# bcsefercik/markerless-robot-camera-calibration

Measured on AMD Instinct MI355X. Metric: point-cloud frames/sec at 200k pts/frame, higher is better.
Workload: dtype f32

## Files before the change

### include/sv_hip.h

```cpp
#ifndef SV_HIP_H
#define SV_HIP_H

#include <stddef.h>
#include <stdint.h>

#ifdef __cplusplus
extern "C" {
#endif

#define SV_OK 0
#define SV_ERR_INVALID (-1)
#define SV_ERR_WORKSPACE (-2)
#define SV_ERR_HIP (-3)
#define SV_ERR_RANGE (-4)
#define SV_ERR_UNSUPPORTED (-5)

#define SV_ACT_NONE 0
#define SV_ACT_RELU 1
#define SV_ACT_LEAKY_RELU 2

#define SV_POOL_MAX 0
#define SV_POOL_AVG 1

#define SV_REDUCE_MEAN 0
#define SV_REDUCE_FIRST 1

#define SV_TILE_ROWS 128
#define SV_COORD_BIAS 131072
#define SV_COORD_BITS 18
#define SV_MAX_BATCH 1024

typedef void* sv_stream_t;

const char* sv_last_error(void);
#define SV_ABI_VERSION 4
int sv_abi_version(void);

size_t sv_voxelize_workspace_bytes(int64_t N);
int sv_voxelize(const void* coords4, int coords_are_int, int64_t N, void* workspace, size_t workspace_bytes,
                uint64_t* keys, int32_t* vcoords, int64_t* inverse, int32_t* order, int32_t* seg_start,
                int32_t* counters, sv_stream_t stream);

int sv_voxel_reduce(const float* feats, int C, const int32_t* order, const int32_t* seg_start, int64_t V, int mode,
                    float* out, sv_stream_t stream);

int sv_hash_build(const uint64_t* keys, int64_t V, uint64_t* table_keys, int32_t* table_vals, int64_t capacity,
                  sv_stream_t stream);

size_t sv_stride_map_workspace_bytes(int64_t V_in);
int sv_stride_map(const uint64_t* keys_in, int64_t V_in, int level, void* workspace, size_t workspace_bytes,
                  uint64_t* keys_out, int32_t* vcoords_out, int32_t* parent, int32_t* child_start, int32_t* counters,
                  sv_stream_t stream);

int sv_kernel_map_k3(const int32_t* vcoords, int64_t V, int tensor_stride, int dilation, const uint64_t* table_keys,
                     const int32_t* table_vals, int64_t capacity, int32_t* nbr, int64_t ld, uint32_t* mask,
                     sv_stream_t stream);
int sv_kernel_map_down(const uint64_t* keys_fine, const int32_t* parent, int64_t V_fine, int level, int64_t V_coarse,
                       int32_t* nbr, int64_t ld, uint32_t* mask, sv_stream_t stream);
int sv_kernel_map_up(const uint64_t* keys_fine, const int32_t* parent, int64_t V_fine, int level, int32_t* nbr,
                     int64_t ld, uint32_t* mask, sv_stream_t stream);

size_t sv_plan_workspace_bytes(int64_t V);
int sv_plan_build(const int32_t* nbr, int64_t ld, const uint32_t* mask, int K, int64_t V, int64_t nbr_base, void* workspace,
                  size_t workspace_bytes, int32_t* perm, int32_t* nbr_s, uint32_t* submask, int32_t* tile_order,
                  int64_t Vpad, sv_stream_t stream);

#define SV_FRAME_MAX_LEVELS 8
#define SV_FRAME_MAX_CUTS 4
#define SV_FRAME_K3 1
#define SV_FRAME_DOWN 2
#define SV_FRAME_UP 4
#define SV_FRAME_SPLIT 8
#define SV_FRAME_RECORD 16
#define SV_FRAME_REC_HASH 1
#define SV_FRAME_REC_K3 2
#define SV_FRAME_REC_DOWN 3
#define SV_FRAME_REC_UP 4
#define SV_FRAME_REC_SPLIT 5
size_t sv_frame_maps_arena_bytes(int64_t N, int levels);
size_t sv_frame_maps_scratch_bytes(int64_t N);
int sv_frame_maps(const void* coords4, int coords_are_int, int64_t N, int levels, void* arena, size_t arena_bytes, void* scratch,
                  size_t scratch_bytes, int32_t* counters_host, int64_t* layout, sv_stream_t stream);
size_t sv_frame_plans_arena_bytes(const int64_t* V, int levels, int flags, const int32_t* split_cuts);
size_t sv_frame_plans_scratch_bytes(const int64_t* V, int levels);
int sv_frame_plans(const void* const* keys, const void* const* coords, const void* const* parent, const int64_t* V, int levels,
                   int flags, const int32_t* split_cuts, const void* const* k3_nbr, const void* const* k3_mask, void* arena,
                   size_t arena_bytes, void* scratch, size_t scratch_bytes, int64_t* layout, int max_records, sv_stream_t stream);

int sv_conv_fwd(const float* in, int64_t V_in, int64_t in_ld, int Cin, const float* W, int K, int Cout, const int32_t* perm,
                const int32_t* nbr_s, const uint32_t* submask, const int32_t* tile_order, int64_t V_out, int64_t Vpad,
                const float* scale,
                const float* shift, const float* residual, int64_t res_ld, int act, float slope, float* out,
                int64_t out_ld, sv_stream_t stream);
int sv_conv_fwd_acc(const float* in, int64_t V_in, int64_t in_ld, int Cin, const float* W, int K, int Cout, const int32_t* perm,
                    const int32_t* nbr_s, const uint32_t* submask, const int32_t* tile_order, int64_t V_out, int64_t Vpad,
                    const float* acc_init, int64_t acc_ld, const float* scale, const float* shift, const float* residual,
                    int64_t res_ld, int act, float slope, float* out, int64_t out_ld, sv_stream_t stream);
const char* sv_conv_last_instance(void);
int sv_conv_set_dispatch(double want_scale, double tail_fraction);

int sv_pack_weights_bf16(const float* W, int K, int Cin, int Cout, uint16_t* Wp, sv_stream_t stream);
int sv_conv_fwd_bf16(const float* in, int64_t V_in, int64_t in_ld, int Cin, const uint16_t* Wp, int K, int Cout,
                     const int32_t* perm, const int32_t* nbr_s, const uint32_t* submask, const int32_t* tile_order, int64_t V_out,
                     int64_t Vpad, const float* acc_init, int64_t acc_ld, const float* scale, const float* shift,
                     const float* residual, int64_t res_ld, int act, float slope, float* out, int64_t out_ld, sv_stream_t stream);

size_t sv_conv_wgrad_workspace_bytes(int64_t Vpad, int K, int Cin, int Cout);
int sv_conv_wgrad(const float* in, int64_t V_in, int64_t in_ld, int Cin, const float* dy, int64_t V_out, int64_t dy_ld,
                  int Cout, int K, const int32_t* perm, const int32_t* nbr_s, const uint32_t* submask, int64_t Vpad,
                  int accumulate, void* workspace, size_t workspace_bytes, float* dW, sv_stream_t stream);

size_t sv_conv_wgrad_bf16_workspace_bytes(int64_t Vpad, int K, int Cin, int Cout);
int sv_conv_wgrad_bf16(const float* in, int64_t V_in, int64_t in_ld, int Cin, const float* dy, int64_t V_out, int64_t dy_ld,
                       int Cout, int K, const int32_t* perm, const int32_t* nbr_s, const uint32_t* submask, int64_t Vpad,
                       int accumulate, void* workspace, size_t workspace_bytes, float* dW, sv_stream_t stream);

int sv_affine_act(const float* in, int64_t in_ld, int C, int64_t V, const float* scale, const float* shift,
                  const float* residual, int64_t res_ld, int act, float slope, float* out, int64_t out_ld,
                  sv_stream_t stream);

size_t sv_col_stats_workspace_bytes(int64_t N);
int sv_col_stats(const float* x, int64_t ld, int64_t N, int C, const float* sub, void* workspace, size_t workspace_bytes,
                 float* col_min, float* col_max, double* col_sum, float* max_row_norm, sv_stream_t stream);
int sv_center_scale(const float* x, int64_t ld, int64_t N, int C, const float* sub, const float* div, const float* add,
                    float* out, int64_t out_ld, sv_stream_t stream);

int sv_batch_offsets(const uint64_t* keys, int64_t V, int B, int32_t* batch_start, sv_stream_t stream);
int sv_global_pool(const float* F, int64_t ld, int C, const int32_t* batch_start, int B, int mode, float* out,
                   sv_stream_t stream);
int sv_slice_rows(const float* F, int64_t ld, int C, const int64_t* inverse, int64_t N, float* out,
                  sv_stream_t stream);
int sv_slice_argmax(const float* F, int64_t ld, int C, const int64_t* inverse, int64_t N, int64_t* label,
                    float* conf, sv_stream_t stream);
int sv_key_point_predictions(const float* logits, int64_t ld, int C, int64_t N, float conf_th, void* workspace,
                             size_t workspace_bytes, float* prob, int64_t* idx, int32_t* selected, sv_stream_t stream);

int sv_key_point_predictions_batched(const float* logits, int64_t ld, int C, const int64_t* seg_start_host, int G, float conf_th,
                                     void* workspace, size_t workspace_bytes, float* prob, int64_t* idx, int32_t* selected,
                                     sv_stream_t stream);
size_t sv_topk_workspace_bytes(int64_t N, int k);
int sv_topk_indices(const float* x, int64_t ld, int64_t N, int k, void* workspace, size_t workspace_bytes, int64_t* idx,
                    sv_stream_t stream);

int sv_kabsch_batched(const double* ref, const double* tgt, const int32_t* K, int Kmax, int B, double* R, double* t,
                      double* q_wxyz, sv_stream_t stream);
int sv_quat_avg_batched(const double* Q, const double* w, const int32_t* M, int Mmax, int B, double* out,
                        sv_stream_t stream);
int sv_add_metric_batched(const double* points, const int32_t* P, int Pmax, const double* gt_pose,
                          const double* pred_pose, int B, double* add_out, sv_stream_t stream);

size_t sv_icp_workspace_bytes(int64_t S);
int sv_icp_point2point(const float* src, int64_t S, const float* tgt, int64_t T, const double* init_T,
                       double max_distance, int max_iterations, double rel_fitness, double rel_rmse, void* workspace,
                       size_t workspace_bytes, double* out_T, double* out_stats, sv_stream_t stream);

size_t sv_normals_workspace_bytes(int64_t N, int max_nn);
int sv_estimate_normals(const float* xyz, int64_t N, double radius, int max_nn, void* workspace, size_t workspace_bytes,
                        float* normals, int32_t* counts, sv_stream_t stream);
size_t sv_icp_point2plane_workspace_bytes(int64_t S);
int sv_icp_point2plane(const float* src, int64_t S, const float* tgt, const float* tgt_normals, int64_t T,
                       const double* init_T, double max_distance, int max_iterations, double rel_fitness,
                       double rel_rmse, void* workspace, size_t workspace_bytes, double* out_T, double* out_stats,
                       sv_stream_t stream);

int sv_fps(const float* xyz, int B, int N, int S, const int64_t* start, int64_t* out, sv_stream_t stream);
int sv_ball_query(const float* xyz, const float* new_xyz, int B, int N, int S, double radius, int nsample,
                  int64_t* out, sv_stream_t stream);
#define SV_BQ_MAX_RADII 4
int sv_ball_query_multi(const float* xyz, const float* new_xyz, int B, int N, int S, int R, const double* radii,
                        const int* nsamples, int64_t* const* out, sv_stream_t stream);
int sv_three_nn_interpolate(const float* xyz1, const float* xyz2, const float* points2, int B, int N, int S, int C,
                            float* out, sv_stream_t stream);
int sv_fps_segmented(const float* xyz, const int64_t* offsets, const int64_t* out_offsets, const int64_t* start, int G,
                     int max_n, int64_t* out, sv_stream_t stream);
#define SV_PN_MAX_LAYERS 4
int sv_pointnet_sa(const float* xyz, const float* points, const float* new_xyz, const int64_t* group_idx, int B, int N,
                   int D, int S, int nsample, const float* params, const int* widths, int L, float* out,
                   sv_stream_t stream);
#define SV_PN_MAX_SCALES 4
int sv_pointnet_sa_msg(const float* xyz, const float* points, const float* new_xyz, int B, int N, int D, int S, int R,
                       const int* nsamples, const int64_t* const* group_idx, const float* const* params,
                       const int* widths, const int* nlayers, float* out, sv_stream_t stream);
// ... 29 lines not shown
```

### markerless-robot-camera-calibration_amd/_lib.py

```python
import ctypes
import os
from ctypes import c_char_p, c_double, c_float, c_int, c_int64, c_size_t, c_void_p

import torch

_HERE = os.path.dirname(os.path.abspath(__file__))
ABI_VERSION = 4
LIB_PATH = os.environ.get("SVHIP_LIB") or os.path.join(_HERE, "libsvhip.so")

SV_ACT_NONE, SV_ACT_RELU, SV_ACT_LEAKY_RELU = 0, 1, 2
SV_POOL_MAX, SV_POOL_AVG = 0, 1
SV_REDUCE_MEAN, SV_REDUCE_FIRST = 0, 1
SV_TILE_ROWS = 128
SV_ERR_UNSUPPORTED = -5
SV_PN_MAX_LAYERS = 4
SV_PN_MAX_SCALES = 4
SV_BQ_MAX_RADII = 4
SV_GROUP_SSG, SV_GROUP_MSG = 0, 1
SV_COORD_BIAS = 1 << 17
SV_COORD_BITS = 18
SV_MAX_BATCH = 1024
SV_FRAME_MAX_LEVELS, SV_FRAME_MAX_CUTS, SV_FRAME_RECORD = 8, 4, 16
SV_FRAME_K3, SV_FRAME_DOWN, SV_FRAME_UP, SV_FRAME_SPLIT = 1, 2, 4, 8
SV_FRAME_REC_HASH, SV_FRAME_REC_K3, SV_FRAME_REC_DOWN, SV_FRAME_REC_UP, SV_FRAME_REC_SPLIT = 1, 2, 3, 4, 5


class SvHipError(RuntimeError):
    pass


_P = c_void_p
SIGNATURES = {
    "sv_last_error": (c_char_p, []),
    "sv_abi_version": (c_int, []),
    "sv_voxelize_workspace_bytes": (c_size_t, [c_int64]),
    "sv_voxelize": (c_int, [_P, c_int, c_int64, _P, c_size_t, _P, _P, _P, _P, _P, _P, _P]),
    "sv_voxel_reduce": (c_int, [_P, c_int, _P, _P, c_int64, c_int, _P, _P]),
    "sv_hash_build": (c_int, [_P, c_int64, _P, _P, c_int64, _P]),
    "sv_stride_map_workspace_bytes": (c_size_t, [c_int64]),
    "sv_stride_map": (c_int, [_P, c_int64, c_int, _P, c_size_t, _P, _P, _P, _P, _P, _P]),
    "sv_kernel_map_k3": (c_int, [_P, c_int64, c_int, c_int, _P, _P, c_int64, _P, c_int64, _P, _P]),
    "sv_kernel_map_down": (c_int, [_P, _P, c_int64, c_int, c_int64, _P, c_int64, _P, _P]),
    "sv_kernel_map_up": (c_int, [_P, _P, c_int64, c_int, _P, c_int64, _P, _P]),
    "sv_plan_workspace_bytes": (c_size_t, [c_int64]),
    "sv_plan_build": (c_int, [_P, c_int64, _P, c_int, c_int64, c_int64, _P, c_size_t, _P, _P, _P, _P, c_int64, _P]),
    "sv_conv_fwd": (
        c_int,
        [_P, c_int64, c_int64, c_int, _P, c_int, c_int, _P, _P, _P, _P, c_int64, c_int64, _P, _P, _P, c_int64, c_int,
         c_float, _P, c_int64, _P],
    ),
    "sv_conv_fwd_acc": (
        c_int,
        [_P, c_int64, c_int64, c_int, _P, c_int, c_int, _P, _P, _P, _P, c_int64, c_int64, _P, c_int64, _P, _P, _P, c_int64, c_int,
         c_float, _P, c_int64, _P],
    ),
    "sv_pack_weights_bf16": (c_int, [_P, c_int, c_int, c_int, _P, _P]),
    "sv_conv_fwd_bf16": (
        c_int,
        [_P, c_int64, c_int64, c_int, _P, c_int, c_int, _P, _P, _P, _P, c_int64, c_int64, _P, c_int64, _P, _P, _P, c_int64, c_int,
         c_float, _P, c_int64, _P],
    ),
    "sv_conv_wgrad_workspace_bytes": (c_size_t, [c_int64, c_int, c_int, c_int]),
    "sv_conv_wgrad": (
        c_int,
        [_P, c_int64, c_int64, c_int, _P, c_int64, c_int64, c_int, c_int, _P, _P, _P, c_int64, c_int, _P, c_size_t, _P, _P],
    ),
    "sv_conv_wgrad_bf16_workspace_bytes": (c_size_t, [c_int64, c_int, c_int, c_int]),
    "sv_conv_wgrad_bf16": (
        c_int,
        [_P, c_int64, c_int64, c_int, _P, c_int64, c_int64, c_int, c_int, _P, _P, _P, c_int64, c_int, _P, c_size_t, _P, _P],
    ),
    "sv_conv_last_instance": (c_char_p, []),
    "sv_conv_set_dispatch": (c_int, [c_double, c_double]),
    "sv_frame_maps_arena_bytes": (c_size_t, [c_int64, c_int]),
    "sv_frame_maps_scratch_bytes": (c_size_t, [c_int64]),
    "sv_frame_maps": (c_int, [_P, c_int, c_int64, c_int, _P, c_size_t, _P, c_size_t, _P, _P, _P]),
    "sv_frame_plans_arena_bytes": (c_size_t, [_P, c_int, c_int, _P]),
    "sv_frame_plans_scratch_bytes": (c_size_t, [_P, c_int]),
    "sv_frame_plans": (c_int, [_P, _P, _P, _P, c_int, c_int, _P, _P, _P, _P, c_size_t, _P, c_size_t, _P, c_int, _P]),
    "sv_affine_act": (c_int, [_P, c_int64, c_int, c_int64, _P, _P, _P, c_int64, c_int, c_float, _P, c_int64, _P]),
    "sv_col_stats_workspace_bytes": (c_size_t, [c_int64]),
    "sv_col_stats": (c_int, [_P, c_int64, c_int64, c_int, _P, _P, c_size_t, _P, _P, _P, _P, _P]),
    "sv_center_scale": (c_int, [_P, c_int64, c_int64, c_int, _P, _P, _P, _P, c_int64, _P]),
    "sv_batch_offsets": (c_int, [_P, c_int64, c_int, _P, _P]),
    "sv_global_pool": (c_int, [_P, c_int64, c_int, _P, c_int, c_int, _P, _P]),
    "sv_slice_rows": (c_int, [_P, c_int64, c_int, _P, c_int64, _P, _P]),
    "sv_slice_argmax": (c_int, [_P, c_int64, c_int, _P, c_int64, _P, _P, _P]),
    "sv_key_point_predictions": (c_int, [_P, c_int64, c_int, c_int64, c_float, _P, c_size_t, _P, _P, _P, _P]),
    "sv_key_point_predictions_batched": (c_int, [_P, c_int64, c_int, _P, c_int, c_float, _P, c_size_t, _P, _P, _P, _P]),
    "sv_topk_workspace_bytes": (c_size_t, [c_int64, c_int]),
    "sv_topk_indices": (c_int, [_P, c_int64, c_int64, c_int, _P, c_size_t, _P, _P]),
    "sv_kabsch_batched": (c_int, [_P, _P, _P, c_int, c_int, _P, _P, _P, _P]),
    "sv_quat_avg_batched": (c_int, [_P, _P, _P, c_int, c_int, _P, _P]),
    "sv_add_metric_batched": (c_int, [_P, _P, c_int, _P, _P, c_int, _P, _P]),
    "sv_icp_workspace_bytes": (c_size_t, [c_int64]),
    "sv_icp_point2point": (c_int, [_P, c_int64, _P, c_int64, _P, c_double, c_int, c_double, c_double, _P, c_size_t, _P, _P,
                                   _P]),
    "sv_normals_workspace_bytes": (c_size_t, [c_int64, c_int]),
    "sv_estimate_normals": (c_int, [_P, c_int64, c_double, c_int, _P, c_size_t, _P, _P, _P]),
    "sv_icp_point2plane_workspace_bytes": (c_size_t, [c_int64]),
    "sv_icp_point2plane": (c_int, [_P, c_int64, _P, _P, c_int64, _P, c_double, c_int, c_double, c_double, _P, c_size_t, _P,
                                   _P, _P]),
    "sv_fps": (c_int, [_P, c_int, c_int, c_int, _P, _P, _P]),
    "sv_three_nn_interpolate": (c_int, [_P, _P, _P, c_int, c_int, c_int, c_int, _P, _P]),
    "sv_cluster_workspace_bytes": (c_size_t, [c_int64]),
    "sv_single_linkage_roots": (c_int, [_P, c_int, c_int64, _P, c_int64, c_double, _P, c_size_t, _P, _P, _P]),
    "sv_select_equal": (c_int, [_P, c_int, c_int64, c_int64, _P, _P, _P, _P]),
    "sv_ball_query": (c_int, [_P, _P, c_int, c_int, c_int, c_double, c_int, _P, _P]),
    "sv_fps_segmented": (c_int, [_P, _P, _P, _P, c_int, c_int, _P, _P]),
    "sv_pointnet_sa": (c_int, [_P, _P, _P, _P, c_int, c_int, c_int, c_int, c_int, _P, _P, c_int, _P, _P]),
    "sv_ball_query_multi": (c_int, [_P, _P, c_int, c_int, c_int, c_int, _P, _P, _P, _P]),
    "sv_pointnet_sa_msg": (c_int, [_P, _P, _P, c_int, c_int, c_int, c_int, c_int, _P, _P, _P, _P, _P, _P, _P]),
    "sv_group_rows": (c_int, [_P, _P, _P, _P, c_int, c_int, c_int, c_int, c_int, c_int, c_int, _P, _P]),
    "sv_index_transpose_workspace_bytes": (c_size_t, [c_int, c_int64, c_int]),
    "sv_index_transpose": (c_int, [_P, c_int, c_int, c_int64, c_int, _P, c_size_t, _P, _P, _P]),
    "sv_gather_transpose": (c_int, [_P, _P, _P, _P, c_int64, c_int, c_int, c_int, c_int64, _P, c_int64, _P]),
    "sv_group_max": (c_int, [_P, c_int64, c_int64, c_int, c_int, _P, _P, _P]),
    "sv_group_max_backward": (c_int, [_P, _P, c_int64, c_int, c_int, _P, _P]),
    "sv_three_nn": (c_int, [_P, _P, c_int, c_int, c_int, _P, _P, _P]),
    "sv_three_nn_gather": (c_int, [_P, _P, _P, c_int, c_int, c_int, c_int, _P, _P]),
}

_lib = None


def load():
    global _lib
    if _lib is not None:
        return _lib
    if not os.path.exists(LIB_PATH):
        raise SvHipError(
            f"{LIB_PATH} not found: build it with `python -c 'import __graft_entry__ as g; g.build()'` "
            "(or `make -C markerless-robot-camera-calibration_amd/csrc`). There is no CPU fallback."
        )
    lib = ctypes.CDLL(LIB_PATH)
    lib.sv_abi_version.restype = c_int
    if lib.sv_abi_version() != ABI_VERSION:
        raise SvHipError(f"{LIB_PATH} has C-ABI version {lib.sv_abi_version()}, this package binds version {ABI_VERSION}: "
                         "rebuild it (`python -c 'import __graft_entry__ as g; g.build()'`)")
    for name, (res, args) in SIGNATURES.items():
        fn = getattr(lib, name)
        fn.restype = res
        fn.argtypes = args
    _lib = lib
    return lib


def _check(rc, name):
    if rc != 0:
        msg = _lib.sv_last_error().decode("utf-8", "replace")
        raise SvHipError(f"{name} failed with status {rc}: {msg}")


def ptr(t):
    if t is None:
        return None
# ... 36 lines not shown
```

### markerless-robot-camera-calibration_amd/csrc/sv_conv_special.hip

```cpp
#include <stdio.h>
#include <stdlib.h>
#include <algorithm>
#include <vector>

#include "sv_conv_params.h"

namespace sv {

constexpr int NARROW_ROWS = 64;
template <int C>
__global__ __launch_bounds__(256) void linear_narrow_kernel(ConvParams p) {
  constexpr int ROWS = NARROW_ROWS, COLS = 32, SW = COLS + 1, LPT = ROWS / 32;
  __shared__ float tile[2][ROWS * SW];
  const int tid = threadIdx.x;
  const int64_t row0 = (int64_t)blockIdx.x * ROWS;
  const int Cin = p.Cin;
  const int lr = tid >> 3, lc = (tid & 7) * 4;
  float4 ra[LPT];
  auto load = [&](int c0) {
#pragma unroll
    for (int i = 0; i < LPT; ++i) {
      const int64_t r = row0 + lr + 32 * i;
      const int c = c0 + lc;
      const bool ok = r < p.V_out && c < Cin;
// ... 463 lines not shown
  for (int j = 0; j < CT; ++j) acc[j] = 0.0f;
  int n[KMAX];
#pragma unroll
  for (int k = 0; k < KMAX; ++k) n[k] = (o >= 0 && k < K) ? p.nbr_s[(int64_t)k * p.Vpad + r] : -1;
  constexpr int G = 9;
#pragma unroll
  for (int k0 = 0; k0 < KMAX; k0 += G) {
    float x[G][CIN];
#pragma unroll
    for (int g = 0; g < G; ++g) {
      const float* src = p.in + (n[k0 + g] >= 0 ? (int64_t)n[k0 + g] * p.in_ld : 0);
#pragma unroll
      for (int c = 0; c < CIN; ++c) x[g][c] = src[c];
    }
#pragma unroll
    for (int g = 0; g < G; ++g) {
      const bool has = n[k0 + g] >= 0;
      if (__ballot(has) == 0ull) continue;
      const float* w = w_s + (k0 + g) * CIN * COUT;
      if (has) {
#pragma unroll
        for (int c = 0; c < CIN; ++c) {
#pragma unroll
          for (int j = 0; j < CT; ++j) acc[j] = __builtin_fmaf(x[g][c], w[c * COUT + j], acc[j]);
        }
      }
    }
  }
  if (o < 0) return;
  float* dst = p.out + o * p.out_ld + j0;
#pragma unroll
  for (int j = 0; j < CT; ++j) {
    float v = acc[j];
    if (p.scale)
      v = __builtin_fmaf(v, p.scale[j0 + j], p.shift ? p.shift[j0 + j] : 0.0f);
    else if (p.shift)
      v = v + p.shift[j0 + j];
    if (p.residual) v = v + p.residual[o * p.res_ld + j0 + j];
    if (p.act == SV_ACT_RELU)
      v = v < 0.f ? 0.f : v;
    else if (p.act == SV_ACT_LEAKY_RELU)
      v = v > 0.f ? v : v * p.slope;
    acc[j] = v;
  }
  if ((p.out_ld & 3) == 0 && (((uintptr_t)p.out) & 15) == 0) {
#pragma unroll
    for (int j = 0; j < CT; j += 4) *(float4*)(dst + j) = make_float4(acc[j], acc[j + 1], acc[j + 2], acc[j + 3]);
  } else {
#pragma unroll
    for (int j = 0; j < CT; ++j) dst[j] = acc[j];
  }
}

int launch_conv_first_mfma(const ConvParams& p, hipStream_t stream) {
  const unsigned cap = 768;
  const unsigned groups = (unsigned)(p.Vpad / 64);
  hipLaunchKernelGGL((conv_first_mfma_kernel<32>), dim3(groups > cap ? cap : groups), dim3(256), 0, stream, p);
  SV_LAUNCH_CHECK();
  note_instance("conv_first_mfma_kernel<3, 32>|fast=1,ring=0,full=1");
  return SV_OK;
}

int launch_conv_first_layer(const ConvParams& p, hipStream_t stream) {
  dim3 grid((unsigned)((p.Vpad + 255) / 256), 1);
  hipLaunchKernelGGL((conv_first_layer_kernel<3, 32, 1>), grid, dim3(256), 0, stream, p);
  note_instance("conv_first_layer_kernel<3, 32>|fast=0,ring=0,full=0");
  SV_LAUNCH_CHECK();
  return SV_OK;
}

int launch_linear_narrow(const ConvParams& p, hipStream_t stream) {
  dim3 grid((unsigned)((p.V_out + NARROW_ROWS - 1) / NARROW_ROWS));
  switch (p.Cout) {
    case 1: hipLaunchKernelGGL((linear_narrow_kernel<1>), grid, dim3(256), 0, stream, p); break;
    case 2: hipLaunchKernelGGL((linear_narrow_kernel<2>), grid, dim3(256), 0, stream, p); break;
    case 3: hipLaunchKernelGGL((linear_narrow_kernel<3>), grid, dim3(256), 0, stream, p); break;
    default: hipLaunchKernelGGL((linear_narrow_kernel<4>), grid, dim3(256), 0, stream, p); break;
  }
  note_instance("linear_narrow_kernel<%d>|fast=0,ring=0,full=0", p.Cout < 4 ? p.Cout : 4);
  SV_LAUNCH_CHECK();
  return SV_OK;
}

}
```

### markerless-robot-camera-calibration_amd/model/robotnet_segmentation.py

```python
import torch.nn as nn

from .. import MinkowskiEngine as ME
from .._lib import SV_ACT_LEAKY_RELU
from ..utils import config
from ._select import pose_backbone, segmentation_backbone

EPS = 1e-6


def _classification_head(UNet, default_classes, class_name):
    class _Head(UNet):
        name = "robotnet"

        def __init__(self, in_channels, out_channels=256, D=3, num_classes=None):
            UNet.__init__(self, in_channels, out_channels, D)
            if num_classes is None:
                num_classes = default_classes()
            self.leaky_relu = ME.MinkowskiLeakyReLU()
            self.regression = nn.Sequential(
                ME.MinkowskiOps.MinkowskiLinear(256, 1024),
                ME.MinkowskiLeakyReLU(),
                ME.MinkowskiOps.MinkowskiLinear(1024, num_classes),
            )
            self.sigm = ME.MinkowskiSigmoid()

        def forward(self, x):
            if isinstance(x, tuple):
                x, _joint_angles = x
            slope = self.leaky_relu.negative_slope
            out = UNet.forward(self, x, final_act=SV_ACT_LEAKY_RELU, final_slope=slope)
            out = self.regression[0].forward_fused(out, act=SV_ACT_LEAKY_RELU,
                                                   slope=self.regression[1].negative_slope)
            return self.regression[2].forward_fused(out)

    _Head.__name__ = _Head.__qualname__ = class_name
    return _Head


def make_robotnet_segmentation(backbone=None):
    return _classification_head(segmentation_backbone(backbone), lambda: config.Config().DATA.classes,
                                "RobotNetSegmentation")


def make_robotnet_vote(backbone=None):
    return _classification_head(pose_backbone(backbone, "ROTATION"),
                                lambda: 2 if config.Config().DATA.data_type == "ee_seg" else 4, "RobotNetVote")


RobotNetSegmentation = make_robotnet_segmentation()
```

### markerless-robot-camera-calibration_amd/nn.py

```python
import math
from ctypes import c_float, c_int, c_int64, c_size_t

import numpy as np
import torch
import torch.nn as nn

from . import _lib, profiling
from ._lib import SV_ACT_LEAKY_RELU, SV_ACT_NONE, SV_ACT_RELU, call, ptr, stream_ptr
from .sparse import SparseTensor, SplitPlan

KERNEL_OFFSET_PERMUTATION = None

import os as _os


def _parse_split_rules(text):
    rules = []
    for part in text.split(";"):
        if part.strip():
            rows, _, cuts = part.partition(":")
            cuts = tuple(int(v) for v in cuts.split(",") if v)
            rules.append((int(rows), cuts[0] if len(cuts) == 1 else cuts))
    return sorted(rules, key=lambda r: -r[0])

# ... 500 lines not shown

    def folded(self):
        if self.training:
            raise _lib.SvHipError("MinkowskiBatchNorm: training-mode statistics are out of scope (inference build); "
                                  "call model.eval()")
        ver = _tensor_versions(self.bn.weight, self.bn.bias, self.bn.running_mean, self.bn.running_var)
        if self._folded is None or self._folded_ver != ver:
            self._folded = fold_bn(self.bn)
            self._folded_ver = ver
        return self._folded

    def forward(self, x):
        if self.training or (x.F.requires_grad and torch.is_grad_enabled()):
            return x.new(self.bn(x.F))
        scale, shift = self.folded()
        return x.new(affine_act(x.F, scale, shift))


class MinkowskiReLU(nn.Module):
    def __init__(self, inplace=False):
        super().__init__()

    def forward(self, x):
        if self.training:
            return x.new(torch.relu(x.F)) if isinstance(x, SparseTensor) else torch.relu(x)
        if isinstance(x, SparseTensor):
            return x.new(affine_act(x.F, act=SV_ACT_RELU))
        return affine_act(x, act=SV_ACT_RELU)


class MinkowskiLeakyReLU(nn.Module):
    def __init__(self, negative_slope=0.01, inplace=False):
        super().__init__()
        self.negative_slope = negative_slope

    def forward(self, x):
        if self.training:
            f = torch.nn.functional.leaky_relu
            return (x.new(f(x.F, self.negative_slope)) if isinstance(x, SparseTensor) else f(x, self.negative_slope))
        if isinstance(x, SparseTensor):
            return x.new(affine_act(x.F, act=SV_ACT_LEAKY_RELU, slope=self.negative_slope))
        return affine_act(x, act=SV_ACT_LEAKY_RELU, slope=self.negative_slope)


class MinkowskiSigmoid(nn.Module):
    def forward(self, x):
        return x.new(torch.sigmoid(x.F))


class MinkowskiLinear(_Bf16Weights, nn.Module):
    def __init__(self, in_features, out_features, bias=True):
        super().__init__()
        self.linear = nn.Linear(in_features, out_features, bias=bias)
        self._wt = None
        self._wt_ver = None
        self.compute_precision = "fp32"
        self.training_precision = "fp32"

    def weight3(self):
        ver = _tensor_versions(self.linear.weight)
        if self._wt is None or self._wt_ver != ver:
            self._wt = self.linear.weight.detach().t().contiguous().unsqueeze(0)
            self._wt_ver = ver
        return self._wt

    def packed_weights_bf16(self):
        return self._packed_bf16(self.linear.weight, self.weight3())

    def forward_fused(self, x, act=SV_ACT_NONE, slope=0.01):
        F = x.F if isinstance(x, SparseTensor) else x
        if self.training:
            out = linear_train(self.linear, F, act, slope, layer=self)
            return x.new(out) if isinstance(x, SparseTensor) else out
        shift = self.linear.bias.detach() if self.linear.bias is not None else None
        wp = self._weight_bf16()
        bf16 = {} if wp is None else {"weight_bf16": wp}
        out = conv_forward(F, self.weight3(), None, F.shape[0], None, shift, None, act, slope, **bf16)
        return x.new(out) if isinstance(x, SparseTensor) else out

    def forward(self, x):
        return self.forward_fused(x)


class MinkowskiGlobalMaxPooling(nn.Module):
    def forward(self, x):
        if self.training:
            return PooledTensor(global_pool_train(x, _lib.SV_POOL_MAX))
        return PooledTensor(global_pool(x, _lib.SV_POOL_MAX))


class MinkowskiGlobalAvgPooling(nn.Module):
    def forward(self, x):
        if self.training:
            return PooledTensor(global_pool_train(x, _lib.SV_POOL_AVG))
        return PooledTensor(global_pool(x, _lib.SV_POOL_AVG))


class PooledTensor:

    def __init__(self, feats):
        self._F = feats

    @property
    def F(self):
        return self._F

    features = F


class BasicBlock(nn.Module):
    expansion = 1
    NORM_TYPE = "BN"

    def __init__(self, inplanes, planes, stride=1, dilation=1, downsample=None, bn_momentum=0.1, dimension=-1):
        super().__init__()
        assert dimension > 0
        self.conv1 = MinkowskiConvolution(inplanes, planes, kernel_size=3, stride=stride, dilation=dilation,
                                          dimension=dimension)
        self.norm1 = MinkowskiBatchNorm(planes, momentum=bn_momentum)
        self.conv2 = MinkowskiConvolution(planes, planes, kernel_size=3, stride=1, dilation=dilation,
                                          dimension=dimension)
        self.norm2 = MinkowskiBatchNorm(planes, momentum=bn_momentum)
        self.relu = MinkowskiReLU(inplace=True)
        self.downsample = downsample

    def forward(self, x):
        out = self.conv1.forward_fused(x, bn=self.norm1, act=SV_ACT_RELU)
        if self.downsample is not None:
            ds_conv, ds_bn = self.downsample[0], self.downsample[1]
            residual = ds_conv.forward_fused(x, bn=ds_bn)
        else:
            residual = x
        return self.conv2.forward_fused(out, bn=self.norm2, residual=residual, act=SV_ACT_RELU)


class Bottleneck(nn.Module):
    expansion = 4
    NORM_TYPE = "BN"

    def __init__(self, inplanes, planes, stride=1, dilation=1, downsample=None, bn_momentum=0.1, dimension=-1):
        super().__init__()
        assert dimension > 0
        self.conv1 = MinkowskiConvolution(inplanes, planes, kernel_size=1, dimension=dimension)
        self.norm1 = MinkowskiBatchNorm(planes, momentum=bn_momentum)
        self.conv2 = MinkowskiConvolution(planes, planes, kernel_size=3, stride=stride, dilation=dilation,
                                          dimension=dimension)
        self.norm2 = MinkowskiBatchNorm(planes, momentum=bn_momentum)
        self.conv3 = MinkowskiConvolution(planes, planes * self.expansion, kernel_size=1, dimension=dimension)
        self.norm3 = MinkowskiBatchNorm(planes * self.expansion, momentum=bn_momentum)
        self.relu = MinkowskiReLU(inplace=True)
        self.downsample = downsample

    def forward(self, x):
        out = self.conv1.forward_fused(x, bn=self.norm1, act=SV_ACT_RELU)
        out = self.conv2.forward_fused(out, bn=self.norm2, act=SV_ACT_RELU)
        if self.downsample is not None:
            residual = self.downsample[0].forward_fused(x, bn=self.downsample[1])
        else:
            residual = x
        return self.conv3.forward_fused(out, bn=self.norm3, residual=residual, act=SV_ACT_RELU)


def kaiming_normal_(tensor, mode="fan_out", nonlinearity="relu"):
    if tensor.dim() == 3:
        K, cin, cout = tensor.shape
    else:
# ... 7 lines not shown
```

### markerless-robot-camera-calibration_amd/profiling.py

```python
import math

import torch

TIMER = None
INSTANCE_LOG = None
TRAIN_LOG = None

_CANDIDATES = {
    "wide3": [(64, 4, 3, 2500), (32, 4, 3, 1500), (32, 2, 3, 0)],
    "wide3_128": [(64, 4, 3, 2500), (64, 4, 2, 1200), (32, 4, 3, 1200), (16, 4, 3, 0)],
    "wide3_128_full": [(64, 4, 3, 2500), (32, 4, 3, 1200), (16, 4, 3, 0)],
    "wide2": [(128, 4, 2, 1300), (64, 4, 2, 1500), (32, 4, 2, 1500), (32, 2, 2, 0)],
    "wide2_64": [(128, 4, 2, 1300), (64, 4, 2, 1500), (32, 4, 2, 1500), (16, 4, 1, 0)],
    "c64": [(64, 4, 1, 1500), (32, 4, 1, 1500), (16, 4, 1, 0)],
    "c32": [(128, 2, 1, 1500), (64, 2, 1, 1500), (32, 2, 1, 0)],
    "c16": [(128, 1, 1, 600), (64, 1, 1, 0)],
}


import os

CONV_TAIL_FRACTION = float(os.environ.get("SV_CONV_TAIL", "0.15"))
CONV_WANT_SCALE = float(os.environ.get("SV_CONV_WANT_SCALE", "0.3"))


_FUSED = {
    (32, 32): [(64, 2, 1, 3000), (32, 2, 1, 0)],
    (32, 64): [(32, 4, 1, 1500), (16, 4, 1, 0)],
    (64, 64): [(32, 4, 1, 1500), (16, 4, 1, 0)],
    (64, 128): [(32, 4, 1, 1500), (16, 4, 1, 0)],
}


def conv_kernel_config(Cout, Vpad, Cin=None, K=1):
    if K == 1 and Cout <= 4 and Cin is not None and Cin >= 64 and Cin % 4 == 0:
        return f"linear_narrow_kernel<{Cout}>"
    if K > 1 and Cin == 3 and Cout == 32:
        return "conv_first_mfma_kernel<3, 32>"
    if K > 1 and Cin == 32 and Cout == 32:
        return "conv_thin_kernel<32, 32>"
    fused = None
    if K > 1 and Cin is not None:
        if Cin == 3 and 16 < Cout <= 32:
            fused = [(64, 2, 1, 3000), (32, 2, 1, 0)]
        else:
            fused = _FUSED.get((Cin, Cout))
    if fused is not None:
        cands = fused
    elif Cout > 128 and (Cout % 192 == 0 or Cout % 96 == 0 or Cout > 2048):
        if Cout % 128 != 0:
            cands = _CANDIDATES["wide3"]
        else:
            cands = _CANDIDATES["wide3_128_full" if (Cin is not None and Cin % 128 == 0) else "wide3_128"]
    elif Cout > 64:
        cands = _CANDIDATES["wide2_64" if Cout % 64 == 0 else "wide2"]
    elif Cout > 32:
        cands = _CANDIDATES["c64"]
    elif Cout > 16:
        cands = _CANDIDATES["c32"]
    else:
        cands = _CANDIDATES["c16"]
    suffix = f", fused {Cin}>" if fused is not None else ">"
    for tm, wn, nt, want in cands:
        tn = wn * nt * 16
        if (Vpad // tm) * ((Cout + tn - 1) // tn) >= want * CONV_WANT_SCALE:
            if ((tm, wn, nt) == (64, 4, 3) and fused is None and K > 1 and Cin is not None and Cin % 4 == 0
                    and Cout % tn == 0 and CONV_TAIL_FRACTION > 0 and int((Vpad // 128) * CONV_TAIL_FRACTION) >= 1):
                return "conv_fwd_dual_kernel<64, 32, 4, 3>"
            return f"conv_fwd_kernel<{tm}, {wn}, {nt}{suffix}"
    tm, wn, nt, _ = cands[-1]
    return f"conv_fwd_kernel<{tm}, {wn}, {nt}{suffix}"


class KernelTimer:
    def __init__(self, capacity=0):
        self.records = []
        self.enabled = True
        self.only = None
        self._pool = [torch.cuda.Event(enable_timing=True) for _ in range(capacity)]
        self._next = 0
        self._first_of_frame = False

    def _event(self):
        if self._next < len(self._pool):
            e = self._pool[self._next]
            self._next += 1
            return e
        return torch.cuda.Event(enable_timing=True)

    def want(self, kernel):
        return self.enabled and (self.only is None or kernel in self.only)

    def start(self):
        e = self._event()
        e.record()
        return e

    def stop(self, start_evt, kernel, K, Cin, Cout, V_out, pairs_dev, level=None, passes=1):
        e = self._event()
        e.record()
        self.records.append((kernel, K, Cin, Cout, V_out, pairs_dev, start_evt, e, self._first_of_frame, level, passes))
        self._first_of_frame = False

    def frame_boundary(self):
        self._first_of_frame = True

    def clear(self):
        self.records = []

    @staticmethod
    def layer_key(kernel, K, Cin, Cout, V_out, level=None):
        where = f"s{level}" if level is not None else f"~2^{int(round(math.log2(max(V_out, 1))))}"
        return (kernel, K, Cin, Cout, where)

    def summarize(self, by_layer=False):
        out = {}
        for kernel, K, Cin, Cout, V_out, pairs_dev, s, e, first, level, passes in self.records:
            if first:
                continue
            P = int(pairs_dev.item()) if pairs_dev is not None else V_out
            ms = s.elapsed_time(e)
            key = self.layer_key(kernel, K, Cin, Cout, V_out, level) if by_layer else kernel
            d = out.setdefault(key, {"launches": 0, "ms": 0.0, "flops": 0.0, "bytes": 0.0, "rows": 0.0, "kernel_launches": 0})
            d["rows"] += V_out
            d["launches"] += 1
            d["kernel_launches"] += passes
            d["ms"] += ms
            d["flops"] += 2.0 * P * Cin * Cout
            d["bytes"] += P * (4.0 * Cin + 8) + 4.0 * V_out * Cout + 4.0 * K * Cin * Cout
        return out


def pass_gflop(fn):
    global TIMER
    saved, TIMER = TIMER, KernelTimer()
    try:
        fn()
        torch.cuda.synchronize()
        return sum(d["flops"] for d in TIMER.summarize().values()) / 1e9
    finally:
        TIMER = saved
```

Measured before the change: 73.99.

## Fuse regression head's two linear layers into one kernel keeping hidden in LDS

Adds a HIP kernel that computes the first linear layer with MFMA, applies bias and leaky ReLU, parks the hidden tile in LDS, and immediately reduces it against the tiny second-layer weights (C≤4). The segmentation head now calls it instead of two separate fused linear launches. This avoids writing and re-reading the V×H hidden activation through global memory and saves a launch. In exchange it adds extra LDS use and a serial per-lane dot product for the second layer, which may limit occupancy.

```diff
diff --git a/include/sv_hip.h b/include/sv_hip.h
--- a/include/sv_hip.h
+++ b/include/sv_hip.h
@@ -98,6 +98,9 @@
                     int64_t res_ld, int act, float slope, float* out, int64_t out_ld, sv_stream_t stream);
 const char* sv_conv_last_instance(void);
 int sv_conv_set_dispatch(double want_scale, double tail_fraction);
+int sv_linear_pair_fwd(const float* x, int64_t V, int64_t x_ld, int Cin, const float* W1, int H, const float* scale1,
+                       const float* shift1, int act1, float slope1, const float* W2, int C, const float* scale2,
+                       const float* shift2, int act2, float slope2, float* out, int64_t out_ld, sv_stream_t stream);
 
 int sv_pack_weights_bf16(const float* W, int K, int Cin, int Cout, uint16_t* Wp, sv_stream_t stream);
 int sv_conv_fwd_bf16(const float* in, int64_t V_in, int64_t in_ld, int Cin, const uint16_t* Wp, int K, int Cout,
diff --git a/markerless-robot-camera-calibration_amd/_lib.py b/markerless-robot-camera-calibration_amd/_lib.py
--- a/markerless-robot-camera-calibration_amd/_lib.py
+++ b/markerless-robot-camera-calibration_amd/_lib.py
@@ -72,6 +72,8 @@
     ),
     "sv_conv_last_instance": (c_char_p, []),
     "sv_conv_set_dispatch": (c_int, [c_double, c_double]),
+    "sv_linear_pair_fwd": (c_int, [_P, c_int64, c_int64, c_int, _P, c_int, _P, _P, c_int, c_float, _P, c_int, _P, _P, c_int,
+                                   c_float, _P, c_int64, _P]),
     "sv_frame_maps_arena_bytes": (c_size_t, [c_int64, c_int]),
     "sv_frame_maps_scratch_bytes": (c_size_t, [c_int64]),
     "sv_frame_maps": (c_int, [_P, c_int, c_int64, c_int, _P, c_size_t, _P, c_size_t, _P, _P, _P]),
diff --git a/markerless-robot-camera-calibration_amd/csrc/sv_conv_special.hip b/markerless-robot-camera-calibration_amd/csrc/sv_conv_special.hip
--- a/markerless-robot-camera-calibration_amd/csrc/sv_conv_special.hip
+++ b/markerless-robot-camera-calibration_amd/csrc/sv_conv_special.hip
@@ -569,4 +569,250 @@
   return SV_OK;
 }
 
-}
+struct PairParams {
+  const float* x;
+  int64_t x_ld, V;
+  int Cin, H;
+  const float *W1, *scale1, *shift1;
+  int act1;
+  float slope1;
+  const float *W2, *scale2, *shift2;
+  int act2;
+  float slope2;
+  float* out;
+  int64_t out_ld;
+  uint32_t w1_bytes;
+};
+constexpr int PAIR_TN = 128;
+constexpr int PAIR_HS = 132;
+constexpr int PAIR_KB = 8;
+static size_t pair_lds_bytes(int tm, int Cin) { return (size_t)(tm * (Cin + 4) + tm * PAIR_HS + 4 * PAIR_TN) * sizeof(float); }
+
+template <int C, int MR>
+__global__ __launch_bounds__(256) void linear_pair_kernel(PairParams p) {
+  constexpr int TM = 16 * MR, TN = PAIR_TN, HS = PAIR_HS, KB = PAIR_KB, QUADS = TN / 4;
+  typedef float bvec_t __attribute__((ext_vector_type(2)));
+  extern __shared__ __attribute__((aligned(16))) float lds[];
+  const int Cin = p.Cin, H = p.H, SA = Cin + 4;
+  float* xs = lds;
+  float* hid = lds + TM * SA;
+  float* w2t = hid + TM * HS;
+  const int tid = threadIdx.x;
+  const int lane = tid & 63;
+  const int wid = __builtin_amdgcn_readfirstlane(tid >> 6);
+  const int li = lane & 15, lq = lane >> 4;
+  const int64_t row0 = (int64_t)blockIdx.x * TM;
+  const int rows = (int)(p.V - row0 < TM ? p.V - row0 : TM);
+  {
+    const float* xg = p.x + row0 * p.x_ld;
+    const int f4 = Cin >> 2, total = TM * f4;
+    for (int e0 = tid; e0 < total; e0 += 4 * 256) {
+      float4 v[4];
+#pragma unroll
+      for (int i = 0; i < 4; ++i) {
+        const int e = e0 + 256 * i, r = e / f4, c = (e - r * f4) * 4;
+        const bool ok = e < total && r < rows;
+        v[i] = ok ? *(const float4*)(xg + (int64_t)r * p.x_ld + c) : make_float4(0.f, 0.f, 0.f, 0.f);
+      }
+#pragma unroll
+      for (int i = 0; i < 4; ++i) {
+        const int e = e0 + 256 * i, r = e / f4, c = (e - r * f4) * 4;
+        if (e < total) *(float4*)(xs + r * SA + c) = v[i];
+      }
+    }
+    for (int e = tid; e < (TM * HS + 4 * TN) / 4; e += 256) ((float4*)hid)[e] = make_float4(0.f, 0.f, 0.f, 0.f);
+  }
+  __syncthreads();
+
+  const __amdgpu_buffer_rsrc_t rsrc_w = __builtin_amdgcn_make_buffer_rsrc((void*)p.W1, 0, (int)p.w1_bytes, 0x00020000);
+  const uint32_t b_voff = (uint32_t)(lq * H + wid * 32 + 2 * li) * 4u;
+  const int nkb = Cin / (4 * KB), ntile = H / TN;
+  auto load_b = [&](int t, int kb, bvec_t (&dst)[KB]) {
+    const uint32_t soff = ((uint32_t)(kb * 4 * KB) * (uint32_t)H + (uint32_t)(t * TN)) * 4u;
+#pragma unroll
+    for (int ks = 0; ks < KB; ++ks) dst[ks] = buffer_load_floats<2>(rsrc_w, b_voff, soff + (uint32_t)(4 * ks) * (uint32_t)H * 4u);
+  };
+  const int j = wid < C ? wid : C - 1;
+  const int crow = lane & (TM - 1);
+  const float* h_lane = hid + crow * HS;
+  const float* w_lane = w2t + j * TN;
+  float cacc = 0.0f;
+  auto chain_quad = [&](int q) {
+    const float4 hv = *(const float4*)(h_lane + 4 * q);
+    const float4 wv = *(const float4*)(w_lane + 4 * q);
+    cacc = __builtin_fmaf(hv.x, wv.x, cacc);
+    cacc = __builtin_fmaf(hv.y, wv.y, cacc);
+    cacc = __builtin_fmaf(hv.z, wv.z, cacc);
+    cacc = __builtin_fmaf(hv.w, wv.w, cacc);
+  };
+
+  f32x4 acc[MR][2];
+#pragma unroll
+  for (int s = 0; s < MR; ++s)
+#pragma unroll
+    for (int n = 0; n < 2; ++n) acc[s][n] = (f32x4){0.f, 0.f, 0.f, 0.f};
+  const float* a_lane = xs + li * SA + lq;
+  float a_cur[MR], a_nx1[MR];
+#pragma unroll
+  for (int s = 0; s < MR; ++s) {
+    a_cur[s] = a_lane[s * 16 * SA];
+    a_nx1[s] = a_lane[s * 16 * SA + 4];
+  }
+  bvec_t b[KB], bn[KB];
+  load_b(0, 0, b);
+  float sc[2] = {1.0f, 1.0f}, sh[2] = {-0.0f, -0.0f};
+  float w2r[(C * TN + 255) / 256];
+  const float slope1 = p.slope1;
+  int t = 0, kb = 0;
+  const int nblk = nkb * ntile;
+  for (int blk = 0; blk < nblk; ++blk) {
+    const bool tile_end = kb == nkb - 1;
+    int kb_n = tile_end ? 0 : kb + 1, t_n = tile_end ? t + 1 : t;
+    if (t_n == ntile) {
+      t_n = t;
+      kb_n = kb;
+    }
+    load_b(t_n, kb_n, bn);
+    if (tile_end) {
+      const int col = t * TN + wid * 32 + 2 * li;
+#pragma unroll
+      for (int n = 0; n < 2; ++n) {
+        sc[n] = p.scale1 ? p.scale1[col + n] : 1.0f;
+        sh[n] = p.shift1 ? p.shift1[col + n] : (p.scale1 ? 0.0f : -0.0f);
+      }
+#pragma unroll
+      for (int i = 0; i < (C * TN + 255) / 256; ++i) {
+        const int e = tid + 256 * i;
+        w2r[i] = e < C * TN ? p.W2[(int64_t)(t * TN + (e & (TN - 1))) * C + (e >> 7)] : 0.0f;
+      }
+    }
+    const float* a_blk = a_lane + kb * (4 * KB);
+    const float* a_nblk = a_lane + (tile_end ? 0 : kb + 1) * (4 * KB);
+#pragma unroll
+    for (int ks = 0; ks < KB; ++ks) {
+      float a_nx2[MR];
+#pragma unroll
+      for (int s = 0; s < MR; ++s)
+        a_nx2[s] = ks + 2 < KB ? a_blk[s * 16 * SA + 4 * (ks + 2)] : a_nblk[s * 16 * SA + 4 * (ks + 2 - KB)];
+#pragma unroll
+      for (int s = 0; s < MR; ++s)
+#pragma unroll
+        for (int n = 0; n < 2; ++n) acc[s][n] = __builtin_amdgcn_mfma_f32_16x16x4f32(a_cur[s], b[ks][n], acc[s][n], 0, 0, 0);
+      if ((ks & 1) == 0) chain_quad(kb * (KB / 2) + ks / 2);
+#pragma unroll
+      for (int s = 0; s < MR; ++s) {
+        a_cur[s] = a_nx1[s];
+        a_nx1[s] = a_nx2[s];
+      }
+    }
+#pragma unroll
+    for (int ks = 0; ks < KB; ++ks) b[ks] = bn[ks];
+    if (tile_end) {
+      for (int q = nkb * (KB / 2); q < QUADS; ++q) chain_quad(q);
+      __syncthreads();
+      auto park = [&](auto act_tag) {
+        constexpr int ACT = decltype(act_tag)::value;
+#pragma unroll
+        for (int s = 0; s < MR; ++s)
+#pragma unroll
+          for (int reg = 0; reg < 4; ++reg) {
+            float2 y;
+            float* yy = &y.x;
+#pragma unroll
+            for (int n = 0; n < 2; ++n) {
+              float v = __builtin_fmaf(acc[s][n][reg], sc[n], sh[n]);
+              if constexpr (ACT == SV_ACT_RELU)
+                v = v < 0.f ? 0.f : v;
+              else if constexpr (ACT == SV_ACT_LEAKY_RELU)
+                v = v > 0.f ? v : v * slope1;
+              yy[n] = v;
+            }
+            *(float2*)(hid + (s * 16 + lq * 4 + reg) * HS + wid * 32 + 2 * li) = y;
+          }
+      };
+      if (p.act1 == SV_ACT_RELU)
+        park(std::integral_constant<int, SV_ACT_RELU>{});
+      else if (p.act1 == SV_ACT_LEAKY_RELU)
+        park(std::integral_constant<int, SV_ACT_LEAKY_RELU>{});
+      else
+        park(std::integral_constant<int, SV_ACT_NONE>{});
+#pragma unroll
+      for (int i = 0; i < (C * TN + 255) / 256; ++i) {
+        const int e = tid + 256 * i;
+        if (e < C * TN) w2t[e] = w2r[i];
+      }
+#pragma unroll
+      for (int s = 0; s < MR; ++s)
+#pragma unroll
+        for (int n = 0; n < 2; ++n) acc[s][n] = (f32x4){0.f, 0.f, 0.f, 0.f};
+      __syncthreads();
+    }
+    t = t_n;
+    kb = kb_n;
+  }
+  for (int q = 0; q < QUADS; ++q) chain_quad(q);
+  const int64_t r = row0 + crow;
+  if (wid >= C || lane >= TM || crow >= rows) return;
+  float v = cacc;
+  if (p.scale2)
+    v = __builtin_fmaf(v, p.scale2[j], p.shift2 ? p.shift2[j] : 0.0f);
+  else if (p.shift2)
+    v = v + p.shift2[j];
+  if (p.act2 == SV_ACT_RELU)
+    v = v < 0.f ? 0.f : v;
+  else if (p.act2 == SV_ACT_LEAKY_RELU)
+    v = v > 0.f ? v : v * p.slope2;
+  p.out[r * p.out_ld + j] = v;
+}
+
+template <int C, int MR>
+static int launch_linear_pair_as(const PairParams& p, hipStream_t stream) {
+  const size_t lds = pair_lds_bytes(16 * MR, p.Cin);
+  static size_t lds_set = 0;
+  if (lds > lds_set) {
+    SV_HIP(hipFuncSetAttribute((const void*)linear_pair_kernel<C, MR>, hipFuncAttributeMaxDynamicSharedMemorySize, (int)lds));
+    lds_set = lds;
+  }
+  const unsigned grid = (unsigned)((p.V + 16 * MR - 1) / (16 * MR));
+  hipLaunchKernelGGL((linear_pair_kernel<C, MR>), dim3(grid), dim3(256), lds, stream, p);
+  note_instance("linear_pair_kernel<%d>|fast=1,ring=0,full=1", C);
+  SV_LAUNCH_CHECK();
+  return SV_OK;
+}
+
+template <int MR>
+static int launch_linear_pair(const PairParams& p, int C, hipStream_t stream) {
+  switch (C) {
+    case 1: return launch_linear_pair_as<1, MR>(p, stream);
+    case 2: return launch_linear_pair_as<2, MR>(p, stream);
+    case 3: return launch_linear_pair_as<3, MR>(p, stream);
+    default: return launch_linear_pair_as<4, MR>(p, stream);
+  }
+}
+
+}
+
+using namespace sv;
+
+extern "C" int sv_linear_pair_fwd(const float* x, int64_t V, int64_t x_ld, int Cin, const float* W1, int H, const float* scale1,
+                                  const float* shift1, int act1, float slope1, const float* W2, int C, const float* scale2,
+                                  const float* shift2, int act2, float slope2, float* out, int64_t out_ld, sv_stream_t stream_) {
+  if (Cin < 32 || Cin > 256 || Cin % 32 != 0 || H < PAIR_TN || H % PAIR_TN != 0 || C < 1 || C > 4) {
+    set_error("sv_linear_pair_fwd: needs Cin a multiple of 32 up to 256, H a multiple of 128, C in 1..4 (got %d, %d, %d)", Cin, H, C);
+    return SV_ERR_UNSUPPORTED;
+  }
+  SV_CHECK_ARG(V >= 0 && x_ld >= Cin && out_ld >= C, "bad rows / row strides");
+  SV_CHECK_ARG(act1 >= SV_ACT_NONE && act1 <= SV_ACT_LEAKY_RELU && act2 >= SV_ACT_NONE && act2 <= SV_ACT_LEAKY_RELU, "bad activation");
+  if (V == 0) return SV_OK;
+  SV_CHECK_ARG(x && W1 && W2 && out, "null pointer");
+  SV_CHECK_ARG(x_ld % 4 == 0 && (((uintptr_t)x) & 15) == 0 && (((uintptr_t)W1) & 7) == 0, "x must be 16-byte aligned with x_ld % 4 == 0, W1 8-byte aligned");
+  SV_CHECK_ARG((V + 15) / 16 < 0x7fffffffll, "too many rows for one launch");
+  PairParams p;
+  p.x = x; p.x_ld = x_ld; p.V = V; p.Cin = Cin; p.H = H;
+  p.W1 = W1; p.scale1 = scale1; p.shift1 = shift1; p.act1 = act1; p.slope1 = slope1;
+  p.W2 = W2; p.scale2 = scale2; p.shift2 = shift2; p.act2 = act2; p.slope2 = slope2;
+  p.out = out; p.out_ld = out_ld;
+  p.w1_bytes = (uint32_t)((uint64_t)Cin * (uint64_t)H * 4u);
+  SV_CHECK_ARG((uint64_t)Cin * (uint64_t)H * 4u < BUF_LIMIT, "W1 too large");
+  return launch_linear_pair<2>(p, C, (hipStream_t)stream_);
+}
diff --git a/markerless-robot-camera-calibration_amd/model/robotnet_segmentation.py b/markerless-robot-camera-calibration_amd/model/robotnet_segmentation.py
--- a/markerless-robot-camera-calibration_amd/model/robotnet_segmentation.py
+++ b/markerless-robot-camera-calibration_amd/model/robotnet_segmentation.py
@@ -2,6 +2,7 @@
 
 from .. import MinkowskiEngine as ME
 from .._lib import SV_ACT_LEAKY_RELU
+from ..nn import linear_pair_forward
 from ..utils import config
 from ._select import pose_backbone, segmentation_backbone
 
@@ -29,9 +30,8 @@
                 x, _joint_angles = x
             slope = self.leaky_relu.negative_slope
             out = UNet.forward(self, x, final_act=SV_ACT_LEAKY_RELU, final_slope=slope)
-            out = self.regression[0].forward_fused(out, act=SV_ACT_LEAKY_RELU,
-                                                   slope=self.regression[1].negative_slope)
-            return self.regression[2].forward_fused(out)
+            return linear_pair_forward(self.regression[0], self.regression[2], out, act=SV_ACT_LEAKY_RELU,
+                                       slope=self.regression[1].negative_slope)
 
     _Head.__name__ = _Head.__qualname__ = class_name
     return _Head
diff --git a/markerless-robot-camera-calibration_amd/nn.py b/markerless-robot-camera-calibration_amd/nn.py
--- a/markerless-robot-camera-calibration_amd/nn.py
+++ b/markerless-robot-camera-calibration_amd/nn.py
@@ -606,6 +606,47 @@
         return self.forward_fused(x)
 
 
+_CONV_FORWARD = conv_forward
+LINEAR_PAIR = _os.environ.get("MRCC_LINEAR_PAIR", "1") != "0"
+
+
+def _linear_pair_ok(first, second, F):
+    if not LINEAR_PAIR or first.training or second.training or torch.is_grad_enabled():
+        return False
+    if first._weight_bf16() is not None or second._weight_bf16() is not None:
+        return False
+    if conv_forward is not _CONV_FORWARD:
+        return False
+    H, Cin = first.linear.weight.shape
+    C = second.linear.weight.shape[0]
+    return (F.is_cuda and F.dtype == torch.float32 and F.dim() == 2 and F.shape[1] == Cin and F.is_contiguous()
+            and F.data_ptr() % 16 == 0 and Cin % 32 == 0 and 32 <= Cin <= 256 and H % 128 == 0 and 1 <= C <= 4
+            and second.linear.weight.shape[1] == H)
+
+
+def linear_pair_forward(first, second, x, act=SV_ACT_NONE, slope=0.01):
+    F = x.F if isinstance(x, SparseTensor) else x
+    if not _linear_pair_ok(first, second, F):
+        return second.forward_fused(first.forward_fused(x, act=act, slope=slope))
+    V, Cin = F.shape
+    w1, w2 = first.weight3(), second.weight3()
+    H, C = w1.shape[2], w2.shape[2]
+    b1 = first.linear.bias.detach() if first.linear.bias is not None else None
+    b2 = second.linear.bias.detach() if second.linear.bias is not None else None
+    out = torch.empty((V, C), dtype=torch.float32, device=F.device)
+    timer = profiling.TIMER
+    kname = profiling.pair_kernel_config(C)
+    t0 = timer.start() if timer is not None and timer.want(kname) else None
+    call("sv_linear_pair_fwd", ptr(F), c_int64(V), c_int64(F.stride(0)), c_int(Cin), ptr(w1), c_int(H), None, ptr(b1),
+         c_int(act), c_float(slope), ptr(w2), c_int(C), None, ptr(b2), c_int(SV_ACT_NONE), c_float(0.01), ptr(out),
+         c_int64(out.stride(0)), stream_ptr())
+    if profiling.INSTANCE_LOG is not None:
+        profiling.INSTANCE_LOG.append((*_lib.conv_last_instance(), 1, Cin, H, V))
+    if t0 is not None:
+        timer.stop(t0, kname, 1, Cin, H, V, None)
+    return x.new(out) if isinstance(x, SparseTensor) else out
+
+
 class MinkowskiGlobalMaxPooling(nn.Module):
     def forward(self, x):
         if self.training:
diff --git a/markerless-robot-camera-calibration_amd/profiling.py b/markerless-robot-camera-calibration_amd/profiling.py
--- a/markerless-robot-camera-calibration_amd/profiling.py
+++ b/markerless-robot-camera-calibration_amd/profiling.py
@@ -72,6 +72,17 @@
     return f"conv_fwd_kernel<{tm}, {wn}, {nt}{suffix}"
 
 
+PAIR_KERNEL = "linear_pair_kernel<"
+
+
+def pair_kernel_config(C):
+    return f"{PAIR_KERNEL}{C}>"
+
+
+def _pair_classes(kernel):
+    return int(kernel[len(PAIR_KERNEL):-1]) if kernel.startswith(PAIR_KERNEL) else None
+
+
 class KernelTimer:
     def __init__(self, capacity=0):
         self.records = []
@@ -126,6 +137,11 @@
             d["launches"] += 1
             d["kernel_launches"] += passes
             d["ms"] += ms
+            C = _pair_classes(kernel)
+            if C is not None:
+                d["flops"] += 2.0 * P * (Cin * Cout + Cout * C)
+                d["bytes"] += 4.0 * P * Cin + 4.0 * V_out * C + 4.0 * (Cin * Cout + Cout * C)
+                continue
             d["flops"] += 2.0 * P * Cin * Cout
             d["bytes"] += P * (4.0 * Cin + 8) + 4.0 * V_out * Cout + 4.0 * K * Cin * Cout
         return out
```

Result: no change. 73.89 (-0.1%).
